# recursiveGecko/Formula-VAD

Measured on AMD Instinct MI355X. Metric: 20ms audio frames/sec end-to-end VAD pipeline, higher is better.
Workload: dtype f32

## Files before the change

### formula-vad_amd/csrc/engine.cpp

```cpp
#include <algorithm>
#include <cctype>
#include <cmath>
#include <cstdio>
#include <cstdlib>
#include <cstring>
#include <atomic>
#include <mutex>
#include <thread>

#include "internal.h"

#ifndef FVAD_DIAG
#define FVAD_DIAG 0
#endif

namespace fvad {

int set_err(const fvad_ctx* ctx, int code, const std::string& msg)
{
    if (ctx) ctx->err = msg;
    return code;
}
int hip_fail(const fvad_ctx* ctx, hipError_t e, const char* what)
{
// ... 60 lines not shown
                    if ((long long)p * p > m) p = m;
                }
                m /= p;
                if (nf >= 14) { hipFree(pd.d); return set_err(ctx, FVAD_ERR_INVALID_FFT_SIZE, "fft_size has too many prime factors"); }
                pd.plan.fac[nf++] = p;
            }
            pd.plan.n_fac = nf;
        }
        it = ctx->vad_plans.emplace(key, pd).first;
        ctx->ws.generation++;
    }
    *out = it->second.plan;
    return FVAD_OK;
}

static int apply_option(fvad_ctx* ctx, const std::string& name, const char* value)
{
    Tuning& tn = ctx->tune;
    const Tuning def;
    const bool unset = !value || !*value;
    const std::string v = unset ? "" : value;
    auto to_long = [&](long& out) { char* end = nullptr; out = strtol(v.c_str(), &end, 10); return end && *end == 0; };
    auto to_bool = [&](bool& out) { if (unset || v == "0") { out = false; return true; } if (v == "1") { out = true; return true; } return false; };
    if (name == "nn_math") {
        if (unset) tn.nn_math_force = -1;
        else if (v == "f32") tn.nn_math_force = FVAD_NN_MATH_F32;
        else if (v == "f16x3") tn.nn_math_force = FVAD_NN_MATH_F16X3;
        else if (v == "bf16x3") tn.nn_math_force = FVAD_NN_MATH_BF16X3;
        else return FVAD_ERR_INVALID_ARGUMENT;
    } else if (name == "gru_kernel") {
        if (!unset && v != "v3w12" && v != "v3w8" && v != "v3w4" && v != "v4w8" && v != "v5w0" && v != "v6w0") return FVAD_ERR_INVALID_ARGUMENT;
        tn.gru_kernel = v;
    } else if (name == "gemm_kernel") {
        if (!unset && v != "v1" && v != "v3" && v != "v3nofold") return FVAD_ERR_INVALID_ARGUMENT;
        tn.gemm_kernel = v;
    } else if (name == "h3_waves") {
        long w = 0;
        if (!unset && (!to_long(w) || (w != 0 && w != 8 && w != 12))) return FVAD_ERR_INVALID_ARGUMENT;
        tn.h3_waves = (int)w;
    } else if (name == "max_chunks") {
        long c = def.max_chunks;
        if (!unset && (!to_long(c) || c < 1)) return FVAD_ERR_INVALID_ARGUMENT;
        tn.max_chunks = c;
    } else if (name == "copy_threads") {
        long c = def.copy_threads;
        if (!unset && (!to_long(c) || c < 1 || c > 256)) return FVAD_ERR_INVALID_ARGUMENT;
        tn.copy_threads = (int)c;
    } else if (name == "ws_spin_ticks") {
        if (unset) { tn.ws_spin_ticks = def.ws_spin_ticks; tn.ws_spin_auto = true; }
        else {
            char* end = nullptr;
            tn.ws_spin_ticks = strtoull(v.c_str(), &end, 10);
            if (!end || *end) return FVAD_ERR_INVALID_ARGUMENT;
            tn.ws_spin_auto = false;
        }
    } else if (name == "ws2_variant") {
        long c = 0;
        if (!unset && (!to_long(c) || c < 0 || c >= (1 << 24))) return FVAD_ERR_INVALID_ARGUMENT;
#if !FVAD_DIAG
        if (c & (1 | 2 | 4 | 32 | 64 | 256 | 512 | 4096 | 8192 | 16384)) return FVAD_ERR_INVALID_ARGUMENT;
#endif
        tn.ws2_variant = (int)c;
    } else if (name == "ws2_waits") {
        long c = 0;
        if (!unset && (!to_long(c) || c < 0 || c > 0x7FFFFFFFL)) return FVAD_ERR_INVALID_ARGUMENT;
        tn.ws2_waits = (unsigned)c;
    } else if (name == "ws2_calibrate") {
// ... 655 lines not shown
```

### formula-vad_amd/csrc/kernels.h

```cpp
#pragma once
#include <hip/hip_runtime.h>
#include <stddef.h>
#include <stdint.h>

#include "../../include/fvad.h"

enum { FVAD_ACT_NONE = 0, FVAD_ACT_RELU = 1, FVAD_ACT_SIGMOID = 2 };

constexpr int kNFft = 320;
constexpr int kNHop = 160;
constexpr int kFramesPerChunk = 50;
constexpr int kWarmupRows = 4;
constexpr int kRowsPerChunk = kFramesPerChunk + kWarmupRows;
constexpr int kNBins = 161;
constexpr int kFeatStride = 176;
constexpr int kDown = 3;
constexpr int kChunk48 = kFramesPerChunk * kNHop * kDown;
constexpr int kVadFft = 1024;
constexpr int kVadFftMax = 16384;

struct LaneCarry {
    float in_tail[kNHop * kDown];
    float feat_tail[kWarmupRows * kNBins];
    float ola_tail[kNHop];
// ... 24 lines not shown
    const float* win320;
    const float* win320n;
    const float* tw160;
    const float* st320;
};

struct VadFftPlan {
    int n;
    const float* win;
    const float* tw;
    const float* st;
    float norm;
    int generic;
    int n_fac;
    int fac[14];
};

int fvad_launch_panel_gemm(const float* A, int lda, const float* Wfrag, const float* bias, float* C,
                           int ldc, long rows, int nt, int n_blocks, int S_steps, int act,
                           int map_T, int map_skip, hipStream_t stream, int n_valid_tiles = 0,
                           const unsigned* guard = nullptr);
struct GemmRowMap {
    int n_rows = 0, L = 0, in_T = 0, in_t0 = 0, out_T = 0, out_t0 = 0;
};
int fvad_launch_panel_gemm_s_rows(const float* A, int lda, const float* Wfrag, const float* bias, float* C, int ldc,
                                  GemmRowMap rm, int nt, int n_blocks, int S_steps, int act, hipStream_t stream,
                                  int n_valid_tiles = 0, const unsigned* guard = nullptr);
int fvad_launch_panel_gemm_s(const float* A, int lda, const float* Wfrag, const float* bias, float* C, int ldc,
                             long rows, int nt, int n_blocks, int S_steps, int act, int map_T, int map_skip,
                             hipStream_t stream, int n_valid_tiles = 0, const unsigned* guard = nullptr);
int fvad_launch_panel_gemm3(const float* A, int lda, const float* Wfrag, const float* bias, float* C,
                            int ldc, long rows, int nt, int n_blocks, int S_steps, int K, int act,
                            int n_valid_tiles, int map_T, int map_skip, int n_wg, hipStream_t stream);
int fvad_launch_panel_gemm_h3(const float* A, int in_ts, int a_ld, const float* Wfrag, const float* bias, float* C,
                              int out, int c_ld, int seq_T, long row_tiles, int nt, int n_blocks, int K, int act,
                              int n_valid_tiles, int map_T, int map_skip, float sx, float sw, float out_sx, int n_wg,
                              hipStream_t stream);
int fvad_launch_gru_rec_h3(const float* gi, const float* Rfrag, const float* bR, float* hsplit,
                           long n_seq_pad, int T, int waves, float sx, float sw, hipStream_t stream);
int fvad_launch_gru_ws2_fallback(float* gi, const float* feat, const float* W1frag_nt2, const float* bG1, const float* R1frag, const float* bR1,
                                 const float* W2frag_nt2, const float* bW2, const float* R2frag, const float* bR2, float* h1, float* h2,
                                 long n_seq_pad, int T, unsigned* sync, unsigned long long* fallbacks, hipStream_t stream,
                                 int zero_at = 0, int zero_n = 0);
int fvad_launch_gru_lat(const float* gi, const float* R2frag, const float* bR, float* hout,
                        long n_seq_pad, int T, const unsigned* guard, int tile_major, hipStream_t stream, int row_tiles = 1);
void fvad_launch_zero_words(unsigned* p, int n, hipStream_t stream);
void fvad_launch_count_word(unsigned long long* counter, const unsigned* word, hipStream_t stream);
bool fvad_gru_ws_shape(long n_seq_pad, int n_cu, int* RT, int* G);
size_t fvad_gru_ws_exchange_floats(long n_seq_pad);
int fvad_launch_gru_ws(const float* gi, const float* R2frag, const float* bR, float* hout, float* hx, unsigned* flags,
                       unsigned* err, long n_seq_pad, int T, int n_cu, int tile_major, unsigned long long spin_ticks,
                       hipStream_t stream);
bool fvad_gru_ws2_shape(long n_seq_pad, int n_cu, int* RT, int* G);
size_t fvad_gru_ws2_exchange_floats(long n_seq_pad);
bool fvad_gru_ws2_gi1_in_kernel(long n_seq_pad, int T, int n_cu, int variant);
bool fvad_gru_ws2_ok(long n_seq_pad, int T, int n_cu, int variant);
const char* fvad_gru_ws2_kernel_name(long n_seq_pad, int T, int n_cu, int variant);
int fvad_launch_gru_ws2(const float* gi1, const float* feat, const float* W1frag, const float* bG1, const float* R1frag, const float* bR1,
                        const float* W2frag, const float* bW2, const float* R2frag, const float* bR2, float* hout2, float* hx,
                        unsigned* flags, unsigned* err, long n_seq_pad, int T, int n_cu, unsigned long long spin_ticks, int variant,
                        unsigned waits, hipStream_t stream, unsigned* lsync = nullptr);
constexpr int kWs2LocalWords = 336;
bool fvad_gru_ws2_local_layer1(long n_seq_pad, int T, int n_cu, int variant);
int fvad_gru_ws2_wait_class(long n_seq_pad, int T, int n_cu, int variant);
unsigned fvad_gru_ws2_builtin_waits(int wait_class, bool local_layer1 = false);
int fvad_launch_gru_gen(const float* gi, int gi_ld, const float* R2frag, const float* bR, float* hout, int h_ld,
// ... 120 lines not shown
```

### formula-vad_amd/csrc/kernels_nn.hip

```cpp

#include <hip/hip_runtime.h>
#include <stdint.h>
#include <type_traits>

#include "kernels.h"

#include "nn_device.h"

__device__ __forceinline__ float act_sigmoid(float x) { return 1.0f / (1.0f + expf(-x)); }

template <int NT, int ACT, int WAVES>
__global__ __launch_bounds__(WAVES * 64) void panel_gemm_kernel(
    const float* __restrict__ A, int lda, const float* __restrict__ Wfrag,
    const float* __restrict__ bias, float* __restrict__ C, int ldc, int S_steps, int row_map_T,
    int row_map_skip, int n_valid_tiles, const unsigned* guard)
{
    __shared__ __attribute__((aligned(16))) float slab[2][NT * 256];
    if (guard && *guard == 0) return;

    const int tid = threadIdx.x;
    const int lane = tid & 63;
    const int wave = tid >> 6;
    const int m = lane & 15;
    const int q = lane >> 4;
// ... 250 lines not shown
                               bias, C, ldc, rm, n_valid_tiles, guard);                                              \
        else                                                                                                         \
            return -1;                                                                                               \
        return 0;                                                                                                    \
    }
    CASES(11, FVAD_ACT_NONE)
    CASES(25, FVAD_ACT_NONE)
    CASES(25, FVAD_ACT_RELU)
    CASES(38, FVAD_ACT_RELU)
    CASES(38, FVAD_ACT_SIGMOID)
#undef CASES
    return -1;
}

template <int T, int N> struct StaticFor {
    template <class F> static __device__ __forceinline__ void run(F&& f) {
        f(std::integral_constant<int, T>{});
        StaticFor<T + 1, N>::run(f);
    }
};
template <int N> struct StaticFor<N, N> {
    template <class F> static __device__ __forceinline__ void run(F&&) {}
};

template <int OFF> __device__ __forceinline__ void lds_read_b128(f32x4& dst, unsigned addr)
{
    asm volatile("ds_read_b128 %0, %1 offset:%2" : "=v"(dst) : "v"(addr), "n"(OFF));
}
template <int N> __device__ __forceinline__ void lds_wait(f32x4& dst)
{
    asm volatile("s_waitcnt lgkmcnt(%1)" : "+v"(dst) : "n"(N));
}

template <int NT, int RT, int ACT, int SP, int WAVES>
__global__ __launch_bounds__(WAVES * 64) __attribute__((amdgpu_waves_per_eu(2, 2))) void panel_gemm3_kernel(
    const float* __restrict__ A, int lda, const float* __restrict__ Wfrag,
    const float* __restrict__ bias, float* __restrict__ C, int ldc, int S_steps, int n_blocks,
    int n_valid_tiles, int row_map_T, int row_map_skip, unsigned n_items, int tail_r)
{
    __shared__ __attribute__((aligned(16))) float slab[2][NT * SP * 256];
    __shared__ __attribute__((aligned(16))) float sbias[2][NT * 16];
    typedef __attribute__((address_space(3))) float lds_float;

    const int tid = threadIdx.x;
    const int lane = tid & 63;
    const int wave = __builtin_amdgcn_readfirstlane(tid >> 6);
    const int m = lane & 15;
    const int q = lane >> 4;
    const int P = (S_steps + SP - 1) / SP;
    constexpr int WAITN = (NT - 1 < 15) ? NT - 1 : 15;

    auto a_pointer = [&](unsigned item, int rt) -> const float* {
        const unsigned panel = item / (unsigned)n_blocks;
        const unsigned row = ((panel * WAVES + wave) * RT + rt) * 16 + m;
        unsigned a_row = row;
        if (row_map_T > 0) {
            const unsigned per = (unsigned)(row_map_T - row_map_skip);
            const unsigned qd = row / per;
            a_row = qd * (unsigned)row_map_T + (unsigned)row_map_skip + (row - qd * per);
        }
        return A + (size_t)a_row * (size_t)lda + 4 * q;
    };
    auto issue = [&](unsigned item, int p, float* dst) {
        const int nblk = (int)(item % (unsigned)n_blocks);
        const int s0 = p * SP;
        const int cnt = (S_steps - s0 < SP) ? (S_steps - s0) : SP;
        const float* src = Wfrag + ((size_t)nblk * S_steps + s0) * (NT * 256);
// ... 13 lines not shown
    };

    unsigned item = (gridDim.x % 8u == 0u) ? (blockIdx.x % 8u) * (gridDim.x / 8u) + blockIdx.x / 8u : blockIdx.x;
    if (item >= n_items) return;
    const unsigned slab_addr[2] = {(unsigned)(uintptr_t)(lds_float*)slab[0] + (unsigned)lane * 16u,
                                   (unsigned)(uintptr_t)(lds_float*)slab[1] + (unsigned)lane * 16u};
    typedef const __attribute__((address_space(1))) f32x4* gptr4;
    const float* a_ptr[RT];
    f32x4 a0[RT], apre[RT];
#pragma unroll
    for (int rt = 0; rt < RT; ++rt) {
        a_ptr[rt] = a_pointer(item, rt);
        a0[rt] = *(gptr4)(a_ptr[rt]);
        apre[rt] = *(gptr4)(a_ptr[rt] + 16);
    }
    issue(item, 0, slab[0]);
    stage_bias(item, sbias[0]);
    __syncthreads();
    int buf = 0, bbuf = 0;

    for (; item < n_items; item += gridDim.x) {
        const unsigned next_item = item + gridDim.x;
        const bool has_next = next_item < n_items;
        f32x4 acc[RT][NT];
        {
            const f32x4* bl = reinterpret_cast<const f32x4*>(sbias[bbuf]) + q;
#pragma unroll
            for (int t = 0; t < NT; ++t) {
                const f32x4 b4 = bl[4 * t];
#pragma unroll
                for (int rt = 0; rt < RT; ++rt) acc[rt][t] = b4;
            }
        }
        const float* a_nextitem[RT];
#pragma unroll
        for (int rt = 0; rt < RT; ++rt) a_nextitem[rt] = has_next ? a_pointer(next_item, rt) : a_ptr[rt];

        for (int p = 0; p < P; ++p) {
            const int s0 = p * SP;
            const int cnt = (S_steps - s0 < SP) ? (S_steps - s0) : SP;
            if (p + 1 < P) issue(item, p + 1, slab[buf ^ 1]);
            else if (has_next) { issue(next_item, 0, slab[buf ^ 1]); stage_bias(next_item, sbias[bbuf ^ 1]); }

            unsigned rd = slab_addr[buf];
            f32x4 w[NT];
            StaticFor<0, NT>::run([&](auto tc) {
                constexpr int t = decltype(tc)::value;
                lds_read_b128<t * 1024>(w[t], rd);
            });
            auto super_step = [&](int s, auto last_c) {
                constexpr bool LAST = decltype(last_c)::value;
                const int sg = s0 + s;
                f32x4 a1[RT];
                if (sg == 0) {
#pragma unroll
                    for (int rt = 0; rt < RT; ++rt) a1[rt] = apre[rt];
                } else {
#pragma unroll
                    for (int rt = 0; rt < RT; ++rt)
                        a1[rt] = *(gptr4)((sg + 1 < S_steps) ? a_ptr[rt] + 16 * (sg + 1) : a_nextitem[rt]);
                }
                const int nr = (sg + 1 < S_steps) ? 4 : tail_r;
                auto mfmas = [&](auto tc) {
                    constexpr int t = decltype(tc)::value;
#pragma unroll
                    for (int rt = 0; rt < RT; ++rt) acc[rt][t] = MFMA16(w[t].x, a0[rt].x, acc[rt][t]);
                    if (nr > 1) {
#pragma unroll
                        for (int rt = 0; rt < RT; ++rt) acc[rt][t] = MFMA16(w[t].y, a0[rt].y, acc[rt][t]);
                    }
                    if (nr > 2) {
#pragma unroll
                        for (int rt = 0; rt < RT; ++rt) acc[rt][t] = MFMA16(w[t].z, a0[rt].z, acc[rt][t]);
                    }
                    if (nr > 3) {
#pragma unroll
                        for (int rt = 0; rt < RT; ++rt) acc[rt][t] = MFMA16(w[t].w, a0[rt].w, acc[rt][t]);
                    }
                };
                StaticFor<0, NT>::run([&](auto tc) {
                    constexpr int t = decltype(tc)::value;
                    if constexpr (LAST) {
                        lds_wait<((NT - 1 - t) < 15 ? (NT - 1 - t) : 15)>(w[t]);
                        mfmas(tc);
                    } else {
                        lds_wait<WAITN>(w[t]);
                        mfmas(tc);
                        lds_read_b128<(NT + t) * 1024>(w[t], rd);
                    }
                });
                rd += NT * 1024;
#pragma unroll
                for (int rt = 0; rt < RT; ++rt) a0[rt] = a1[rt];
            };
            for (int s = 0; s + 1 < cnt; ++s) super_step(s, std::false_type{});
            super_step(cnt - 1, std::true_type{});
            __syncthreads();
// ... 25 lines not shown
            o.z = __int_as_float(__builtin_amdgcn_ds_bpermute(bp_addr, __float_as_int(v[2])));
            o.w = __int_as_float(__builtin_amdgcn_ds_bpermute(bp_addr, __float_as_int(v[3])));
            *reinterpret_cast<f32x4*>(c_ptr[rt] + 16 * t) = o;
        };
        if (valid_t >= NT) {
#pragma unroll
            for (int t = 0; t < NT; ++t)
#pragma unroll
                for (int rt = 0; rt < RT; ++rt) emit(t, rt);
        } else {
#pragma unroll
            for (int t = 0; t < NT; ++t) {
                if (t < valid_t) {
#pragma unroll
                    for (int rt = 0; rt < RT; ++rt) emit(t, rt);
                }
            }
        }
        bbuf ^= 1;
#pragma unroll
        for (int rt = 0; rt < RT; ++rt) a_ptr[rt] = a_nextitem[rt];
    }
}

int fvad_launch_panel_gemm3(const float* A, int lda, const float* Wfrag, const float* bias, float* C,
                            int ldc, long rows, int nt, int n_blocks, int S_steps, int K, int act,
                            int n_valid_tiles, int map_T, int map_skip, int n_wg, hipStream_t stream)
{
    if (rows % 256) return -1;
    const int n_last = K - 16 * (S_steps - 1);
    const int tail_r = n_last >= 4 ? 4 : (n_last < 1 ? 4 : n_last);
    const unsigned n_items = (unsigned)((rows / 256) * n_blocks);
    const unsigned grid = n_items < (unsigned)n_wg ? n_items : (unsigned)n_wg;
#define CASE3(NT_, ACT_, SP_)                                                                         \
    if (nt == NT_ && act == ACT_) {                                                                   \
        hipLaunchKernelGGL((panel_gemm3_kernel<NT_, 2, ACT_, SP_, 8>), dim3(grid), dim3(512), 0, stream, \
                           A, lda, Wfrag, bias, C, ldc, S_steps, n_blocks, n_valid_tiles, map_T,      \
                           map_skip, n_items, tail_r);                                                \
        return 0;                                                                                     \
    }
    CASE3(15, FVAD_ACT_NONE, 5)
    CASE3(13, FVAD_ACT_RELU, 5)
    CASE3(11, FVAD_ACT_SIGMOID, 6)
#undef CASE3
    return -1;
}


template <int WAVES>
__device__ __forceinline__ void gru3_issue_slab(const float* __restrict__ src, float* lds_dst, int wave, unsigned lane16)
{
    asm volatile("" : "+v"(lane16));
#pragma unroll
    for (int b = wave; b < 3 * GRU_J; b += WAVES) {
        __builtin_amdgcn_global_load_lds(
            (const __attribute__((address_space(1))) void*)((const __attribute__((address_space(1))) char*)src + b * 1024 + lane16),
            (__attribute__((address_space(3))) void*)(lds_dst + b * 256), 16, 0, 0);
    }
}

template <int WAVES, int D, bool TS3>
__global__ __launch_bounds__(WAVES * 64) void gru_rec3_kernel(const float* __restrict__ gi,
                                                              const float* __restrict__ R2frag,
                                                              const float* __restrict__ bR,
                                                              float* hout, int T, float* hs3)
{
    __shared__ __attribute__((aligned(16))) float slab[2][GRU2_SLAB];
    typedef __attribute__((address_space(3))) float lds_float;

    const int tid = threadIdx.x;
    const int lane = tid & 63;
    const int wave = __builtin_amdgcn_readfirstlane(tid >> 6);
    const int m = lane & 15;
    const int q = lane >> 4;
    typedef const __attribute__((address_space(1))) char* gbytes;
    const size_t seq0 = (size_t)(blockIdx.x * WAVES + wave) * 16;
    gbytes gi_w = (gbytes)(gi + seq0 * T * (3 * GRU_H));
// ... 548 lines not shown
```

### formula-vad_amd/csrc/nn_dispatch.cpp

```cpp
#include <algorithm>
#include <atomic>
#include <cmath>
#include <cstdio>
#include <cstdlib>
#include <cstring>
#include <mutex>
#include <thread>

#include "internal.h"

namespace fvad {

void free_workspace_nn(Workspace& ws)
{
    float** bufs[] = {&ws.feat, &ws.spec, &ws.a1, &ws.gi, &ws.h1, &ws.h2, &ws.hs1, &ws.hs2, &ws.f2, &ws.f3, &ws.gains};
    for (float** b : bufs) { if (*b) hipFree(*b); *b = nullptr; }
    if (ws.descs) hipFree(ws.descs);
    if (ws.h_descs) hipHostFree(ws.h_descs);
    ws.descs = nullptr; ws.h_descs = nullptr;
    ws.descs_mirror.clear();
    ws.cap_chunks = 0;
    ws.cap_rows = 0;
    ws.a1_cap_rows = ws.h_cap_rows = ws.hs_cap_rows = 0;
}
// ... 292 lines not shown
    auto S = [](int K) { return (K + 15) / 16; };
    int rc = 0;
    ctx->last_nn_path = "f32: panel_gemm<8> + gru_gen (model dims " + std::to_string(g.F1) + "/" + std::to_string(g.H) + "/" +
                        std::to_string(g.N2) + "/" + std::to_string(g.N3) + ")";
    time_begin(ctx, "fc1_gemm");
    rc |= fvad_launch_panel_gemm(ws.feat, kFeatStride, m.g_fc1_w.p, m.g_fc1_b.p, ws.a1, g.F1p, rows, 8, g.F1p / 128, S(161), FVAD_ACT_NONE, 0, 0, st);
    time_end(ctx);
    time_begin(ctx, "gru1_in_gemm");
    rc |= fvad_launch_panel_gemm(ws.a1, g.F1p, m.g_gi1_w.p, m.g_gi1_b.p, ws.gi, g.Gp, rows, 8, g.Gp / 128, S(g.F1), FVAD_ACT_NONE, 0, 0, st);
    time_end(ctx);
    time_begin(ctx, "gru1_rec");
    rc |= fvad_launch_gru_gen(ws.gi, g.Gp, m.g_r1.p, m.g_br1.p, ws.h1, g.Hp, n_pad, T, g.J, st);
    time_end(ctx);
    time_begin(ctx, "gru2_in_gemm");
    rc |= fvad_launch_panel_gemm(ws.h1, g.Hp, m.g_gi2_w.p, m.g_gi2_b.p, ws.gi, g.Gp, rows, 8, g.Gp / 128, g.J, FVAD_ACT_NONE, 0, 0, st);
    time_end(ctx);
    time_begin(ctx, "gru2_rec");
    rc |= fvad_launch_gru_gen(ws.gi, g.Gp, m.g_r2.p, m.g_br2.p, ws.h2, g.Hp, n_pad, T, g.J, st);
    time_end(ctx);
    time_begin(ctx, "fc2_gemm");
    rc |= fvad_launch_panel_gemm(ws.h2, g.Hp, m.g_fc2_w.p, m.g_fc2_b.p, ws.f2, g.N2p, rows_out, 8, g.N2p / 128, g.J, FVAD_ACT_RELU, skip ? T : 0, skip, st);
    time_end(ctx);
    time_begin(ctx, "fc3_gemm");
    rc |= fvad_launch_panel_gemm(ws.f2, g.N2p, m.g_fc3_w.p, m.g_fc3_b.p, ws.f3, g.N3p, rows_out, 8, g.N3p / 128, S(g.N2), FVAD_ACT_RELU, 0, 0, st);
    time_end(ctx);
    time_begin(ctx, "fc4_gemm");
    rc |= fvad_launch_panel_gemm(ws.f3, g.N3p, m.g_fc4_w.p, m.g_fc4_b.p, ws.gains, kFeatStride, rows_out, 11, 1, S(g.N3), FVAD_ACT_SIGMOID, 0, 0, st);
    time_end(ctx);
    if (rc) return set_err(ctx, FVAD_ERR_INVALID_ARGUMENT, "no kernel instance for this layer shape");
    FVAD_HIP(ctx, hipGetLastError());
    return FVAD_OK;
}

int run_nn(fvad_ctx* ctx, long n_pad, int T, int skip, long n_real)
{
    if (!ctx->dm.loaded) return set_err(ctx, FVAD_ERR_NO_MODEL, "NSNet2 weights not loaded");
    if (n_real <= 0 || n_real > n_pad) n_real = n_pad;
    if (ctx->dm.generic) return run_nn_generic(ctx, n_pad, T, skip);
    Workspace& ws = ctx->ws;
    const DeviceModel& m = ctx->dm;
    hipStream_t st = ctx->stream;
    const long rows = n_pad * T;
    const long rows_out = n_pad * (T - skip);
    int rc = 0;
    const Tuning& tn = ctx->tune;
    const char* force = tn.gemm_kernel.empty() ? nullptr : tn.gemm_kernel.c_str();
    const int math = nn_math_effective(ctx);
    const bool h3 = math == FVAD_NN_MATH_F16X3, b3 = math == FVAD_NN_MATH_BF16X3;
    if ((h3 || b3) && n_pad % 128) return set_err(ctx, FVAD_ERR_INVALID_ARGUMENT, "the emulated kernels need a batch padded to 128 sequences");
    {
        const size_t r = (size_t)rows;
        const bool nofold = force && strstr(force, "nofold");
        if (r > ws.cap_rows || (h3 ? r > ws.hs_cap_rows : r > ws.h_cap_rows) || (nofold && r > ws.a1_cap_rows))
            return set_err(ctx, FVAD_ERR_INVALID_ARGUMENT, "NSNet2 workspace not allocated for this arithmetic / batch");
    }
    if (b3) {
        if (!ws.b3_hs1 || (size_t)n_pad * (size_t)T > ws.b3_cap_rows) return set_err(ctx, FVAD_ERR_INVALID_ARGUMENT, "bf16x3 workspace not allocated");
        auto gemm_b3 = [&](const float* A, int in_ts, int a_ld, const DevBuf& W, const float* b, float* Cc, int out, int c_ld, int seq_T,
                           long row_tiles, int nt, int nblk, int K, int act, int valid, int mT, int mskip) {
            return fvad_launch_panel_gemm_b3(A, in_ts, a_ld, W.p, b, Cc, out, c_ld, seq_T, row_tiles, nt, nblk, K, act, valid, mT, mskip, ctx->n_cu, st);
        };
        const int waves = n_pad % 192 == 0 ? 12 : 8;
        const long G = n_pad / 16;
        ctx->last_nn_path = std::string("bf16x3: panel_gemm_b3 (fc1 folded) + gru_rec3<") + std::to_string(waves) + "> (f32 recurrences)";
        time_begin(ctx, "gru1_in_gemm_fc1folded");
        rc |= gemm_b3(ws.feat, 0, kFeatStride, m.gi1f_b3, m.gi1f_bzr.p, ws.gi, 0, 1200, T, G * T, 15, 5, 161, FVAD_ACT_NONE, 75, 0, 0);
        time_end(ctx);
        time_begin(ctx, "gru1_rec");
        rc |= fvad_launch_gru_rec3(ws.gi, m.r1v2.p, m.br1.p, ws.h1, n_pad, T, waves, st, ws.b3_hs1);
        time_end(ctx);
        time_begin(ctx, "gru2_in_gemm");
        rc |= gemm_b3(ws.b3_hs1, 1, 13, m.gi2_b3, m.gi2_bzr.p, ws.gi, 0, 1200, T, G * T, 15, 5, 400, FVAD_ACT_NONE, 75, 0, 0);
        time_end(ctx);
        time_begin(ctx, "gru2_rec");
        rc |= fvad_launch_gru_rec3(ws.gi, m.r2v2.p, m.br2.p, ws.h2, n_pad, T, waves, st, ws.b3_hs2);
        time_end(ctx);
        time_begin(ctx, "fc2_gemm");
        rc |= gemm_b3(ws.b3_hs2, 1, 13, m.fc2_b3, m.fc2h3_b.p, ws.b3_f2, 2, 19, T - skip, G * (T - skip), 10, 4, 400, FVAD_ACT_RELU, 38, skip ? T : 0, skip);
        time_end(ctx);
        time_begin(ctx, "fc3_gemm");
        rc |= gemm_b3(ws.b3_f2, 1, 19, m.fc3_b3, m.fc3h3_b.p, ws.b3_f3, 2, 19, T - skip, G * (T - skip), 10, 4, 600, FVAD_ACT_RELU, 38, 0, 0);
        time_end(ctx);
        time_begin(ctx, "fc4_gemm");
        rc |= gemm_b3(ws.b3_f3, 1, 19, m.fc4_b3, m.fc4h3_b.p, ws.gains, 0, kFeatStride, T - skip, G * (T - skip), 12, 1, 600, FVAD_ACT_SIGMOID, 11, 0, 0);
        time_end(ctx);
        if (rc) return set_err(ctx, FVAD_ERR_INVALID_ARGUMENT, "no kernel instance for this layer shape");
        FVAD_HIP(ctx, hipGetLastError());
        return FVAD_OK;
    }
    const bool big = h3 || (force ? force[1] != '1' : (tn.reproducible || n_pad >= 2048));
    if (tn.reproducible && !force && (rows % 256 || rows_out % 256))
        return set_err(ctx, FVAD_ERR_INVALID_ARGUMENT, "reproducible: batch not padded to the persistent GEMM's 256-row panels");
    if (big && rows % 256 == 0 && rows_out % 256 == 0) {
        auto gemm = [&](const float* A, int lda, const float* W, const float* b, float* Cc, int ldc, long r, int nt,
                        int nblk, int S, int K, int act, int valid, int mT, int mskip) {
            return fvad_launch_panel_gemm3(A, lda, W, b, Cc, ldc, r, nt, nblk, S, K, act, valid, mT, mskip, ctx->n_cu, st);
        };
        auto gemm_h3 = [&](const float* A, int in_ts, int a_ld, const DevBuf& W, const DeviceModel::H3Scale& sc, const float* b,
                           float* Cc, int out, int c_ld, int seq_T, long row_tiles, int nt, int nblk, int K, int act,
                           int valid, int mT, int mskip, float out_sx) {
            return fvad_launch_panel_gemm_h3(A, in_ts, a_ld, W.p, b, Cc, out, c_ld, seq_T, row_tiles, nt, nblk, K, act, valid,
                                             mT, mskip, sc.sx, sc.sw, out_sx, ctx->n_cu, st);
        };
        if (h3) {
            int waves = n_pad % 192 == 0 ? 12 : 8;
            if ((tn.h3_waves == 8 || tn.h3_waves == 12) && n_pad % (16 * tn.h3_waves) == 0) waves = tn.h3_waves;
            ctx->last_nn_path = std::string("f16x3: panel_gemm_h3 + gru_rec_h3<") + std::to_string(waves) + ">";
            const long G = n_pad / 16;
            time_begin(ctx, "gru1_in_gemm_fc1folded");
            rc |= gemm_h3(ws.feat, 0, kFeatStride, m.gi1f_h3, m.h3_gi1f, m.gi1f_bzr.p, ws.gi, 1, 75, T, G * T, 15, 5, 161, FVAD_ACT_NONE, 75, 0, 0, 1.0f);
            time_end(ctx);
            time_begin(ctx, "gru1_rec");
            rc |= fvad_launch_gru_rec_h3(ws.gi, m.r1_h3.p, m.br1.p, ws.hs1, n_pad, T, waves, m.h3_r1.sx, m.h3_r1.sw, st);
            time_end(ctx);
            time_begin(ctx, "gru2_in_gemm");
            rc |= gemm_h3(ws.hs1, 1, 13, m.gi2_h3, m.h3_gi2, m.gi2_bzr.p, ws.gi, 1, 75, T, G * T, 15, 5, 400, FVAD_ACT_NONE, 75, 0, 0, 1.0f);
            time_end(ctx);
            time_begin(ctx, "gru2_rec");
            rc |= fvad_launch_gru_rec_h3(ws.gi, m.r2_h3.p, m.br2.p, ws.hs2, n_pad, T, waves, m.h3_r2.sx, m.h3_r2.sw, st);
            time_end(ctx);
            time_begin(ctx, "fc2_gemm");
            rc |= gemm_h3(ws.hs2, 1, 13, m.fc2_h3, m.h3_fc2, m.fc2h3_b.p, ws.f2, 2, 19, T - skip, G * (T - skip), 10, 4, 400, FVAD_ACT_RELU, 38, skip ? T : 0, skip, m.h3_fc3.sx);
            time_end(ctx);
            time_begin(ctx, "fc3_gemm");
            rc |= gemm_h3(ws.f2, 1, 19, m.fc3_h3, m.h3_fc3, m.fc3h3_b.p, ws.f3, 2, 19, T - skip, G * (T - skip), 10, 4, 600, FVAD_ACT_RELU, 38, 0, 0, m.h3_fc4.sx);
            time_end(ctx);
            time_begin(ctx, "fc4_gemm");
            rc |= gemm_h3(ws.f3, 1, 19, m.fc4_h3, m.h3_fc4, m.fc4h3_b.p, ws.gains, 0, kFeatStride, T - skip, G * (T - skip), 12, 1, 600, FVAD_ACT_SIGMOID, 11, 0, 0, 1.0f);
            time_end(ctx);
            if (rc) return set_err(ctx, FVAD_ERR_INVALID_ARGUMENT, "no kernel instance for this layer shape");
            FVAD_HIP(ctx, hipGetLastError());
            return FVAD_OK;
        }
        const bool fold = !(force && strstr(force, "nofold"));
        const GruChoice gc = pick_gru(ctx, n_pad, T, fold);
        ctx->last_nn_path = std::string("f32: panel_gemm3") + (fold ? " (fc1 folded)" : "") + " + " +
                            (gc.version == 3 ? "gru_rec3<" + std::to_string(gc.waves) + ">" : gc.version == 5 ? std::string("gru_ws") : std::string("gru_lat"));
        if (gc.version == 5 && (rc = prepare_gru_ws(ctx, n_pad))) return rc;
        const bool bzr = gc.version == 3;
        if (fold) {
            time_begin(ctx, "gru1_in_gemm_fc1folded");
            rc |= gemm(ws.feat, kFeatStride, m.gi1f_w.p, bzr ? m.gi1f_bzr.p : m.gi1f_b.p, ws.gi, 1200, rows, 15, 5, 11, 161, FVAD_ACT_NONE, 75, 0, 0);
            time_end(ctx);
        } else {
            time_begin(ctx, "fc1_gemm");
            rc |= fvad_launch_panel_gemm(ws.feat, kFeatStride, m.fc1_w.p, m.fc1_b.p, ws.a1, 400, rows, 25, 1, 11, FVAD_ACT_NONE, 0, 0, st);
            time_end(ctx);
            time_begin(ctx, "gru1_in_gemm");
            rc |= gemm(ws.a1, 400, m.gi1v2_w.p, m.gi1_btm.p, ws.gi, 1200, rows, 15, 5, 25, 400, FVAD_ACT_NONE, 75, 0, 0);
            time_end(ctx);
        }
        time_begin(ctx, "gru1_rec");
        rc |= launch_gru(ctx, gc, ws.gi, m.r1v2, m.br1.p, ws.h1, n_pad, T, 0, 1);
        time_end(ctx);
        time_begin(ctx, "gru2_in_gemm");
        rc |= gemm(ws.h1, 400, m.gi2v2_w.p, bzr ? m.gi2_bzr.p : m.gi2_btm.p, ws.gi, 1200, rows, 15, 5, 25, 400, FVAD_ACT_NONE, 75, 0, 0);
        time_end(ctx);
        time_begin(ctx, "gru2_rec");
        rc |= launch_gru(ctx, gc, ws.gi, m.r2v2, m.br2.p, ws.h2, n_pad, T, 1, 1);
        time_end(ctx);
        time_begin(ctx, "fc2_gemm");
        rc |= gemm(ws.h2, 400, m.fc2v3_w.p, m.fc2v3_b.p, ws.f2, 608, rows_out, 13, 3, 25, 400, FVAD_ACT_RELU, 38, skip ? T : 0, skip);
        time_end(ctx);
        time_begin(ctx, "fc3_gemm");
        rc |= gemm(ws.f2, 608, m.fc3v3_w.p, m.fc3v3_b.p, ws.f3, 608, rows_out, 13, 3, 38, 600, FVAD_ACT_RELU, 38, 0, 0);
        time_end(ctx);
        time_begin(ctx, "fc4_gemm");
        rc |= gemm(ws.f3, 608, m.fc4_w.p, m.fc4_b.p, ws.gains, kFeatStride, rows_out, 11, 1, 38, 600, FVAD_ACT_SIGMOID, 11, 0, 0);
        time_end(ctx);
        if (rc) return set_err(ctx, FVAD_ERR_INVALID_ARGUMENT, "no kernel instance for this layer shape");
        FVAD_HIP(ctx, hipGetLastError());
        return FVAD_OK;
    }
    const int fam = rows > 2048 ? 1 : 0, snt = fam ? 4 : 2;
    const int nb_gi = (75 + snt - 1) / snt, nb_fc = (38 + snt - 1) / snt;
    const GruChoice gcs = pick_gru(ctx, n_pad, T, false);
    const bool gi1_in_kernel = gcs.version == 6 && fvad_gru_ws2_gi1_in_kernel(n_pad, T, ctx->n_cu, tn.ws2_variant);
    if (!gi1_in_kernel) {
        time_begin(ctx, "gru1_in_gemm_fc1folded");
        rc |= fvad_launch_panel_gemm_s(ws.feat, kFeatStride, m.s_gi1f_w[fam].p, m.gi1f_b.p, ws.gi, 1200, rows, snt, nb_gi, 11, FVAD_ACT_NONE, 0, 0, st, 75);
        time_end(ctx);
    }
    if (gcs.version >= 5 && (rc = prepare_gru_ws(ctx, n_pad))) return rc;
    ctx->last_nn_path = std::string("f32: panel_gemm (fc1 folded) + ") + (gcs.version == 6 ? fvad_gru_ws2_kernel_name(n_pad, T, ctx->n_cu, tn.ws2_variant) :
                        gcs.version == 5 ? "gru_ws" : "gru_lat");
    if (gcs.version == 6) {
        unsigned* err = ws.ws_sync + 512;
        time_begin(ctx, "gru12_rec_pipelined");
        rc |= ws_serialised(ctx, [&] {
            return fvad_launch_gru_ws2(ws.gi, ws.feat, m.s_w1frag.p, m.gi1f_b.p, m.r1v2.p, m.br1.p, m.s_w2frag.p, m.s_bw2.p, m.r2v2.p, m.br2.p, ws.h2,
                                       ws.hx, ws.ws_sync, err, n_pad, T, ctx->n_cu, ws_spin_deadline(ctx, gru_ws2_cost_both_layers(n_pad, T, ctx->n_cu, tn.ws2_variant) * T / 55.0), tn.ws2_variant,
                                       tn.ws2_waits ? tn.ws2_waits : tn.ws2_waits_cal[fvad_gru_ws2_wait_class(n_pad, T, ctx->n_cu, tn.ws2_variant)], st,
                                       ws.ws_sync + kWsLocalAt);
        });
        rc |= fvad_launch_gru_ws2_fallback(ws.gi, gi1_in_kernel ? ws.feat : nullptr, m.s_gi1f_w[0].p, m.gi1f_b.p, m.r1v2.p, m.br1.p, m.s_gi2_w[0].p,
                                           m.gi2_btm.p, m.r2v2.p, m.br2.p, ws.h1, ws.h2, n_pad, T, ws.ws_sync, ws.ws_fallbacks, st, (int)kWsLocalAt, kWs2LocalWords);
        {
            hipStreamCaptureStatus cap = hipStreamCaptureStatusNone;
            (void)hipStreamIsCapturing(st, &cap);
            if (rc == 0 && cap == hipStreamCaptureStatusNone) ws.sync_clean = true;
        }
        time_end(ctx);
// ... 228 lines not shown
            ws.descs_mirror.assign(hd, hd + n);
        }
        time_begin(ctx, "stft320_logpow");
        const int fft_parts = n <= 85 ? 3 : (n <= 128 ? 2 : 1);
        fvad_launch_stft(dd, (int)n, ctx->tb, ws.feat, ws.spec, ctx->stream, fft_parts);
        time_end(ctx);
        for (const Tap& t : taps) {
            const LaneJob& lj = jobs[t.job];
            if (lj.h_spec)
                FVAD_HIP(ctx, hipMemcpyAsync(lj.h_spec + t.chunk0 * (size_t)(kFramesPerChunk * kNBins * 2),
                                             ws.spec + (size_t)t.batch0 * (kFramesPerChunk * kNBins * 2),
                                             t.count * (size_t)(kFramesPerChunk * kNBins * 2) * sizeof(float), hipMemcpyDeviceToHost, ctx->stream));
            if (lj.h_feat)
                FVAD_HIP(ctx, hipMemcpy2DAsync(lj.h_feat + t.chunk0 * (size_t)(kRowsPerChunk * kNBins), kNBins * sizeof(float),
                                               ws.feat + (size_t)t.batch0 * (kRowsPerChunk * kFeatStride), kFeatStride * sizeof(float),
                                               kNBins * sizeof(float), t.count * (size_t)kRowsPerChunk, hipMemcpyDeviceToHost, ctx->stream));
        }
        const long n_pad = padded_batch(ctx, n, kRowsPerChunk, kWarmupRows);
        rc = run_nn(ctx, n_pad, kRowsPerChunk, kWarmupRows, n);
        if (rc) return rc;
        time_begin(ctx, "istft320_ola_up3");
        fvad_launch_istft(dd, (int)n, ctx->tb, ws.spec, ws.gains, kFramesPerChunk, 0, ctx->stream, fft_parts);
        time_end(ctx);
        for (size_t t : touched) jobs[t].cur ^= 1;
        if (n_launches) ++*n_launches;
        job = j;
        chunk_in_job = c;
    }
    FVAD_HIP(ctx, hipGetLastError());
    return FVAD_OK;
}

}
```

Before: 25.05 million.

## Add weight-resident persistent GEMM with balanced panel split for fc1-folded GRU input

Adds a persistent GEMM kernel that loads one column block of weight fragments into LDS once per workgroup and then streams row panels through it. A host-side split spreads workgroups over column blocks in proportion to their tile counts and gives each workgroup a strided set of panels. By default this is used only for the fc1-folded GRU1 input GEMM. It is meant to remove repeated weight reloads from global memory and to balance work across CUs, at the cost of more LDS use and more complex launch logic. The fc2/fc3 panel_gemm3 instance also skips MFMAs on the padding tile in the last block.

```diff
diff --git a/formula-vad_amd/csrc/engine.cpp b/formula-vad_amd/csrc/engine.cpp
--- a/formula-vad_amd/csrc/engine.cpp
+++ b/formula-vad_amd/csrc/engine.cpp
@@ -116,7 +116,7 @@
         if (!unset && v != "v3w12" && v != "v3w8" && v != "v3w4" && v != "v4w8" && v != "v5w0" && v != "v6w0") return FVAD_ERR_INVALID_ARGUMENT;
         tn.gru_kernel = v;
     } else if (name == "gemm_kernel") {
-        if (!unset && v != "v1" && v != "v3" && v != "v3nofold") return FVAD_ERR_INVALID_ARGUMENT;
+        if (!unset && v != "v1" && v != "v3" && v != "v3nofold" && v != "v4" && v != "v4nofold") return FVAD_ERR_INVALID_ARGUMENT;
         tn.gemm_kernel = v;
     } else if (name == "h3_waves") {
         long w = 0;
diff --git a/formula-vad_amd/csrc/kernels.h b/formula-vad_amd/csrc/kernels.h
--- a/formula-vad_amd/csrc/kernels.h
+++ b/formula-vad_amd/csrc/kernels.h
@@ -80,6 +80,17 @@
 int fvad_launch_panel_gemm3(const float* A, int lda, const float* Wfrag, const float* bias, float* C,
                             int ldc, long rows, int nt, int n_blocks, int S_steps, int K, int act,
                             int n_valid_tiles, int map_T, int map_skip, int n_wg, hipStream_t stream);
+constexpr int FVAD_RES_MAX_WG = 320;
+struct GemmResSplit {
+    unsigned p0[FVAD_RES_MAX_WG];
+    unsigned short cnt[FVAD_RES_MAX_WG];
+    unsigned char blk[FVAD_RES_MAX_WG], stride[FVAD_RES_MAX_WG];
+};
+bool fvad_gemm_res_split(GemmResSplit& sp, long n_panels, const int* w, int n_blocks, int n_wg);
+int fvad_panel_gemm_res_rows(int K, int n_valid_tiles, int act);
+int fvad_launch_panel_gemm_res(const float* A, int lda, const float* Wfrag, int src_nt, const float* bias, float* C, int ldc,
+                               long rows, int K, int act, int n_valid_tiles, int map_T, int map_skip, int n_wg,
+                               hipStream_t stream);
 int fvad_launch_panel_gemm_h3(const float* A, int in_ts, int a_ld, const float* Wfrag, const float* bias, float* C,
                               int out, int c_ld, int seq_T, long row_tiles, int nt, int n_blocks, int K, int act,
                               int n_valid_tiles, int map_T, int map_skip, float sx, float sw, float out_sx, int n_wg,
diff --git a/formula-vad_amd/csrc/kernels_nn.hip b/formula-vad_amd/csrc/kernels_nn.hip
--- a/formula-vad_amd/csrc/kernels_nn.hip
+++ b/formula-vad_amd/csrc/kernels_nn.hip
@@ -306,7 +306,7 @@
     asm volatile("s_waitcnt lgkmcnt(%1)" : "+v"(dst) : "n"(N));
 }
 
-template <int NT, int RT, int ACT, int SP, int WAVES>
+template <int NT, int RT, int ACT, int SP, int WAVES, int NTS = NT>
 __global__ __launch_bounds__(WAVES * 64) __attribute__((amdgpu_waves_per_eu(2, 2))) void panel_gemm3_kernel(
     const float* __restrict__ A, int lda, const float* __restrict__ Wfrag,
     const float* __restrict__ bias, float* __restrict__ C, int ldc, int S_steps, int n_blocks,
@@ -386,6 +386,7 @@
                 for (int rt = 0; rt < RT; ++rt) acc[rt][t] = b4;
             }
         }
+        const bool skip_pad = NTS != NT && n_valid_tiles - (int)(item % (unsigned)n_blocks) * NT == NTS;
         const float* a_nextitem[RT];
 #pragma unroll
         for (int rt = 0; rt < RT; ++rt) a_nextitem[rt] = has_next ? a_pointer(next_item, rt) : a_ptr[rt];
@@ -417,6 +418,7 @@
                 const int nr = (sg + 1 < S_steps) ? 4 : tail_r;
                 auto mfmas = [&](auto tc) {
                     constexpr int t = decltype(tc)::value;
+                    if (t >= NTS && skip_pad) return;
 #pragma unroll
                     for (int rt = 0; rt < RT; ++rt) acc[rt][t] = MFMA16(w[t].x, a0[rt].x, acc[rt][t]);
                     if (nr > 1) {
@@ -508,17 +510,290 @@
     const int tail_r = n_last >= 4 ? 4 : (n_last < 1 ? 4 : n_last);
     const unsigned n_items = (unsigned)((rows / 256) * n_blocks);
     const unsigned grid = n_items < (unsigned)n_wg ? n_items : (unsigned)n_wg;
-#define CASE3(NT_, ACT_, SP_)                                                                         \
+#define CASE3(NT_, ACT_, SP_, NTS_)                                                                       \
     if (nt == NT_ && act == ACT_) {                                                                   \
-        hipLaunchKernelGGL((panel_gemm3_kernel<NT_, 2, ACT_, SP_, 8>), dim3(grid), dim3(512), 0, stream, \
+        hipLaunchKernelGGL((panel_gemm3_kernel<NT_, 2, ACT_, SP_, 8, NTS_>), dim3(grid), dim3(512), 0, stream, \
                            A, lda, Wfrag, bias, C, ldc, S_steps, n_blocks, n_valid_tiles, map_T,      \
                            map_skip, n_items, tail_r);                                                \
         return 0;                                                                                     \
     }
-    CASE3(15, FVAD_ACT_NONE, 5)
-    CASE3(13, FVAD_ACT_RELU, 5)
-    CASE3(11, FVAD_ACT_SIGMOID, 6)
+    CASE3(15, FVAD_ACT_NONE, 5, 15)
+    CASE3(13, FVAD_ACT_RELU, 5, 12)
+    CASE3(11, FVAD_ACT_SIGMOID, 6, 11)
 #undef CASE3
+    return -1;
+}
+
+template <int OFF> __device__ __forceinline__ void lds_read_b32(float& dst, unsigned addr)
+{
+    asm volatile("ds_read_b32 %0, %1 offset:%2" : "=v"(dst) : "v"(addr), "n"(OFF));
+}
+template <int N> __device__ __forceinline__ void lds_wait(float& dst)
+{
+    asm volatile("s_waitcnt lgkmcnt(%1)" : "+v"(dst) : "n"(N));
+}
+
+template <int NT, int NTL, int RT, int ACT, int S, int TAIL_R>
+__global__ __launch_bounds__(512) __attribute__((amdgpu_waves_per_eu(2, 2))) void panel_gemm_res_kernel(
+    const float* __restrict__ A, int lda, const float* __restrict__ Wfrag, int src_nt,
+    const float* __restrict__ bias, float* __restrict__ C, int ldc, int n_blocks, int row_map_T, int row_map_skip,
+    GemmResSplit sp)
+{
+    constexpr int WAVES = 8;
+    constexpr bool TAILQ = TAIL_R == 1;
+    constexpr int FULL = TAILQ ? S - 1 : S;
+    static_assert(NT <= 15 && NTL >= 1 && NTL <= NT && FULL >= 2, "lgkmcnt is a 4-bit field; the ring needs two full steps");
+    static_assert((2 * NT - 1) * 1024 < 65536, "ds_read offset field");
+    __shared__ __attribute__((aligned(16))) float wres[FULL * NT * 256 + (TAILQ ? NT * 64 : 0)];
+    __shared__ __attribute__((aligned(16))) float sbias[NT * 16];
+    typedef __attribute__((address_space(3))) float lds_float;
+    typedef const __attribute__((address_space(1))) f32x4* gptr4;
+
+    const int tid = threadIdx.x;
+    const int lane = tid & 63;
+    const int wave = __builtin_amdgcn_readfirstlane(tid >> 6);
+    const int m = lane & 15;
+    const int q = lane >> 4;
+
+    asm volatile("" ::: "a0");
+    const unsigned slot = (gridDim.x % 8u == 0u) ? (blockIdx.x % 8u) * (gridDim.x / 8u) + blockIdx.x / 8u : blockIdx.x;
+    const unsigned cnt = sp.cnt[slot];
+    if (cnt == 0) return;
+    const int nblk = sp.blk[slot];
+    const unsigned stride = sp.stride[slot];
+    const unsigned p_first = sp.p0[slot];
+    const int ntv = (nblk == n_blocks - 1) ? NTL : NT;
+
+    for (int idx = tid; idx < FULL * NT * 64; idx += WAVES * 64) {
+        const int fb = idx >> 6, s = fb / NT, t = fb - s * NT;
+        const int tile = nblk * NT + t, sb = tile / src_nt, st = tile - sb * src_nt;
+        if (t < ntv)
+            reinterpret_cast<f32x4*>(wres)[idx] =
+                reinterpret_cast<const f32x4*>(Wfrag)[((size_t)(sb * S + s) * src_nt + st) * 64 + (idx & 63)];
+    }
+    if (TAILQ) {
+        for (int idx = tid; idx < NT * 64; idx += WAVES * 64) {
+            const int t = idx >> 6;
+            const int tile = nblk * NT + t, sb = tile / src_nt, st = tile - sb * src_nt;
+            if (t < ntv) wres[FULL * NT * 256 + idx] = Wfrag[(((size_t)(sb * S + S - 1) * src_nt + st) * 64 + (idx & 63)) * 4];
+        }
+    }
+    if (tid < ntv * 4) reinterpret_cast<f32x4*>(sbias)[tid] = reinterpret_cast<const f32x4*>(bias + nblk * (NT * 16))[tid];
+    __syncthreads();
+
+    auto a_pointer = [&](unsigned panel, int rt) -> const float* {
+        const unsigned row = ((panel * WAVES + wave) * RT + rt) * 16 + m;
+        unsigned a_row = row;
+        if (row_map_T > 0) {
+            const unsigned per = (unsigned)(row_map_T - row_map_skip);
+            const unsigned qd = row / per;
+            a_row = qd * (unsigned)row_map_T + (unsigned)row_map_skip + (row - qd * per);
+        }
+        return A + (size_t)a_row * (size_t)lda + 4 * q;
+    };
+
+    auto body = [&](auto ntv_c) {
+        constexpr int NTV = decltype(ntv_c)::value;
+        const unsigned base = (unsigned)(uintptr_t)(lds_float*)wres + (unsigned)lane * 16u;
+        const unsigned tbase = (unsigned)(uintptr_t)(lds_float*)(wres + FULL * NT * 256) + (unsigned)lane * 4u;
+        unsigned panel = p_first;
+        const float* a_ptr[RT];
+        f32x4 a0[RT], apre[RT];
+#pragma unroll
+        for (int rt = 0; rt < RT; ++rt) {
+            a_ptr[rt] = a_pointer(panel, rt);
+            a0[rt] = *(gptr4)(a_ptr[rt]);
+            apre[rt] = *(gptr4)(a_ptr[rt] + 16);
+        }
+        f32x4 w[NTV];
+        float wt[NTV];
+        StaticFor<0, NTV>::run([&](auto tc) {
+            constexpr int t = decltype(tc)::value;
+            lds_read_b128<t * 1024>(w[t], base);
+        });
+
+        for (unsigned i = 0; i < cnt; ++i, panel += stride) {
+            const bool has_next = i + 1 < cnt;
+            f32x4 acc[RT][NTV];
+            {
+                unsigned boff = (unsigned)q;
+                asm volatile("" : "+v"(boff));
+                const f32x4* bl = reinterpret_cast<const f32x4*>(sbias) + boff;
+#pragma unroll
+                for (int t = 0; t < NTV; ++t) {
+                    const f32x4 b4 = bl[4 * t];
+#pragma unroll
+                    for (int rt = 0; rt < RT; ++rt) acc[rt][t] = b4;
+                }
+            }
+            unsigned rd = base;
+            auto super_step = [&](int sg, auto mode_c) {
+                constexpr int MODE = decltype(mode_c)::value;
+                constexpr int NR = MODE == 2 ? TAIL_R : 4;
+                f32x4 a1[RT];
+                if (sg == 0) {
+#pragma unroll
+                    for (int rt = 0; rt < RT; ++rt) a1[rt] = apre[rt];
+                } else {
+#pragma unroll
+                    for (int rt = 0; rt < RT; ++rt) a1[rt] = *(gptr4)(MODE == 2 ? a_ptr[rt] : a_ptr[rt] + 16 * (sg + 1));
+                }
+                StaticFor<0, NTV>::run([&](auto tc) {
+                    constexpr int t = decltype(tc)::value;
+                    if constexpr (MODE == 2 && TAILQ) lds_wait<NTV - 1>(wt[t]);
+                    else lds_wait<NTV - 1>(w[t]);
+                    const float wx = (MODE == 2 && TAILQ) ? wt[t] : w[t].x;
+#pragma unroll
+                    for (int rt = 0; rt < RT; ++rt) acc[rt][t] = MFMA16(wx, a0[rt].x, acc[rt][t]);
+                    if constexpr (NR > 1) {
+#pragma unroll
+                        for (int rt = 0; rt < RT; ++rt) acc[rt][t] = MFMA16(w[t].y, a0[rt].y, acc[rt][t]);
+                    }
+                    if constexpr (NR > 2) {
+#pragma unroll
+                        for (int rt = 0; rt < RT; ++rt) acc[rt][t] = MFMA16(w[t].z, a0[rt].z, acc[rt][t]);
+                    }
+                    if constexpr (NR > 3) {
+#pragma unroll
+                        for (int rt = 0; rt < RT; ++rt) acc[rt][t] = MFMA16(w[t].w, a0[rt].w, acc[rt][t]);
+                    }
+                    if constexpr (MODE == 0) lds_read_b128<(NT + t) * 1024>(w[t], rd);
+                    else if constexpr (MODE == 1) lds_read_b32<t * 256>(wt[t], tbase);
+                    else lds_read_b128<t * 1024>(w[t], base);
+                });
+                if (MODE == 0) rd += NT * 1024;
+#pragma unroll
+                for (int rt = 0; rt < RT; ++rt) a0[rt] = a1[rt];
+            };
+            constexpr int N0 = TAILQ ? S - 2 : S - 1;
+            for (int s = 0; s < N0; ++s) super_step(s, std::integral_constant<int, 0>{});
+            if (TAILQ) super_step(S - 2, std::integral_constant<int, 1>{});
+            if (has_next) {
+#pragma unroll
+                for (int rt = 0; rt < RT; ++rt) a_ptr[rt] = a_pointer(panel + stride, rt);
+            }
+            super_step(S - 1, std::integral_constant<int, 2>{});
+
+#pragma unroll
+            for (int rt = 0; rt < RT; ++rt) apre[rt] = *(gptr4)(a_ptr[rt] + 16);
+            const int bp_addr = ((lane >> 2) + 16 * (lane & 3)) * 4;
+            float* c_ptr[RT];
+#pragma unroll
+            for (int rt = 0; rt < RT; ++rt) {
+                const unsigned row = ((panel * WAVES + wave) * RT + rt) * 16 + (unsigned)(lane >> 2);
+                c_ptr[rt] = C + (size_t)row * (size_t)ldc + nblk * (NT * 16) + 4 * (lane & 3);
+            }
+#pragma unroll
+            for (int t = 0; t < NTV; ++t) {
+#pragma unroll
+                for (int rt = 0; rt < RT; ++rt) {
+                    f32x4 v = acc[rt][t];
+                    if (ACT == FVAD_ACT_RELU) {
+                        v.x = fmaxf(v.x, 0.f); v.y = fmaxf(v.y, 0.f); v.z = fmaxf(v.z, 0.f); v.w = fmaxf(v.w, 0.f);
+                    } else if (ACT == FVAD_ACT_SIGMOID) {
+                        v.x = act_sigmoid(v.x); v.y = act_sigmoid(v.y); v.z = act_sigmoid(v.z); v.w = act_sigmoid(v.w);
+                    }
+                    f32x4 o;
+                    o.x = __int_as_float(__builtin_amdgcn_ds_bpermute(bp_addr, __float_as_int(v[0])));
+                    o.y = __int_as_float(__builtin_amdgcn_ds_bpermute(bp_addr, __float_as_int(v[1])));
+                    o.z = __int_as_float(__builtin_amdgcn_ds_bpermute(bp_addr, __float_as_int(v[2])));
+                    o.w = __int_as_float(__builtin_amdgcn_ds_bpermute(bp_addr, __float_as_int(v[3])));
+                    *reinterpret_cast<f32x4*>(c_ptr[rt] + 16 * t) = o;
+                }
+            }
+        }
+        StaticFor<0, NTV>::run([&](auto tc) { lds_wait<0>(w[decltype(tc)::value]); });
+    };
+    if (NTL != NT && ntv != NT) body(std::integral_constant<int, NTL>{});
+    else body(std::integral_constant<int, NT>{});
+}
+
+bool fvad_gemm_res_split(GemmResSplit& sp, long n_panels, const int* w, int n_blocks, int n_wg)
+{
+    if (n_wg > FVAD_RES_MAX_WG || n_blocks < 1 || n_blocks > n_wg || n_blocks > 255 || n_panels <= 0) return false;
+    int N[256], k_next[256];
+    for (int b = 0; b < n_blocks; ++b) { N[b] = 1; k_next[b] = 0; }
+    for (int i = n_blocks; i < n_wg; ++i) {
+        int best = 0;
+        for (int b = 1; b < n_blocks; ++b)
+            if ((long)w[b] * N[best] > (long)w[best] * N[b]) best = b;
+        ++N[best];
+    }
+    int blk_of[FVAD_RES_MAX_WG], k_of[FVAD_RES_MAX_WG];
+    for (int i = 0; i < n_wg; ++i) {
+        int best = -1;
+        for (int b = 0; b < n_blocks; ++b) {
+            if (k_next[b] >= N[b]) continue;
+            if (best < 0 || (long)(2 * k_next[b] + 1) * N[best] < (long)(2 * k_next[best] + 1) * N[b]) best = b;
+        }
+        blk_of[i] = best;
+        k_of[i] = k_next[best]++;
+    }
+    const int nx = n_wg % 8 == 0 ? 8 : 1, per_x = n_wg / nx;
+    for (int x = 0; x < nx; ++x) {
+        int k0[256], n[256];
+        for (int b = 0; b < n_blocks; ++b) { k0[b] = -1; n[b] = 0; }
+        for (int i = x * per_x; i < (x + 1) * per_x; ++i) {
+            if (k0[blk_of[i]] < 0) k0[blk_of[i]] = k_of[i];
+            ++n[blk_of[i]];
+        }
+        for (int i = x * per_x; i < (x + 1) * per_x; ++i) {
+            const int b = blk_of[i], j = k_of[i] - k0[b];
+            const long lo = n_panels * k0[b] / N[b], hi = n_panels * (k0[b] + n[b]) / N[b];
+            const long len = hi - lo, c = len > j ? (len - j + n[b] - 1) / n[b] : 0;
+            if (c > 65535 || n[b] > 255) return false;
+            sp.p0[i] = (unsigned)(lo + j);
+            sp.cnt[i] = (unsigned short)c;
+            sp.blk[i] = (unsigned char)b;
+            sp.stride[i] = (unsigned char)n[b];
+        }
+    }
+    return true;
+}
+
+namespace {
+struct ResInstance { int K, tiles, act, nt, ntl, rt; };
+constexpr ResInstance kResInstances[] = {
+    {161, 75, FVAD_ACT_NONE, 15, 15, 2},
+    {400, 75, FVAD_ACT_NONE, 5, 5, 6},
+    {400, 38, FVAD_ACT_RELU, 5, 3, 6},
+};
+const ResInstance* res_instance(int K, int n_valid_tiles, int act)
+{
+    for (const ResInstance& r : kResInstances)
+        if (r.K == K && r.tiles == n_valid_tiles && r.act == act) return &r;
+    return nullptr;
+}
+}
+
+int fvad_panel_gemm_res_rows(int K, int n_valid_tiles, int act)
+{
+    const ResInstance* r = res_instance(K, n_valid_tiles, act);
+    return r ? 8 * r->rt * 16 : 0;
+}
+
+int fvad_launch_panel_gemm_res(const float* A, int lda, const float* Wfrag, int src_nt, const float* bias, float* C, int ldc,
+                               long rows, int K, int act, int n_valid_tiles, int map_T, int map_skip, int n_wg,
+                               hipStream_t stream)
+{
+    const ResInstance* r = res_instance(K, n_valid_tiles, act);
+    if (!r || rows <= 0 || rows % (8 * r->rt * 16)) return -1;
+    const int n_blocks = (n_valid_tiles + r->nt - 1) / r->nt;
+    int w[16];
+    for (int b = 0; b < n_blocks; ++b) w[b] = b + 1 < n_blocks ? r->nt : r->ntl;
+    if (n_wg > FVAD_RES_MAX_WG) n_wg = FVAD_RES_MAX_WG - FVAD_RES_MAX_WG % 8;
+    GemmResSplit sp;
+    if (n_wg < n_blocks || !fvad_gemm_res_split(sp, rows / (8 * r->rt * 16), w, n_blocks, n_wg)) return -1;
+#define CASE_RES(NT_, NTL_, RT_, ACT_, S_, TAIL_)                                                                    \
+    if (r->nt == NT_ && r->ntl == NTL_ && act == ACT_) {                                                             \
+        hipLaunchKernelGGL((panel_gemm_res_kernel<NT_, NTL_, RT_, ACT_, S_, TAIL_>), dim3(n_wg), dim3(512), 0, stream, A, lda, \
+                           Wfrag, src_nt, bias, C, ldc, n_blocks, map_T, map_skip, sp);                              \
+        return 0;                                                                                                    \
+    }
+    CASE_RES(15, 15, 2, FVAD_ACT_NONE, 11, 1)
+    CASE_RES(5, 5, 6, FVAD_ACT_NONE, 25, 4)
+    CASE_RES(5, 3, 6, FVAD_ACT_RELU, 25, 4)
+#undef CASE_RES
     return -1;
 }
 
diff --git a/formula-vad_amd/csrc/nn_dispatch.cpp b/formula-vad_amd/csrc/nn_dispatch.cpp
--- a/formula-vad_amd/csrc/nn_dispatch.cpp
+++ b/formula-vad_amd/csrc/nn_dispatch.cpp
@@ -348,6 +348,8 @@
     return FVAD_OK;
 }
 
+static bool res_by_default(const char* layer) { return strcmp(layer, "gi1f") == 0; }
+
 int run_nn(fvad_ctx* ctx, long n_pad, int T, int skip, long n_real)
 {
     if (!ctx->dm.loaded) return set_err(ctx, FVAD_ERR_NO_MODEL, "NSNet2 weights not loaded");
@@ -408,8 +410,15 @@
     if (tn.reproducible && !force && (rows % 256 || rows_out % 256))
         return set_err(ctx, FVAD_ERR_INVALID_ARGUMENT, "reproducible: batch not padded to the persistent GEMM's 256-row panels");
     if (big && rows % 256 == 0 && rows_out % 256 == 0) {
-        auto gemm = [&](const float* A, int lda, const float* W, const float* b, float* Cc, int ldc, long r, int nt,
+        const bool v4 = force && force[1] == '4';
+        std::string res_layers;
+        auto gemm = [&](const char* layer, const float* A, int lda, const float* W, const float* b, float* Cc, int ldc, long r, int nt,
                         int nblk, int S, int K, int act, int valid, int mT, int mskip) {
+            const bool want = force ? v4 : res_by_default(layer);
+            if (want && fvad_launch_panel_gemm_res(A, lda, W, nt, b, Cc, ldc, r, K, act, valid, mT, mskip, ctx->n_cu, st) == 0) {
+                res_layers += std::string(res_layers.empty() ? "" : ", ") + layer;
+                return 0;
+            }
             return fvad_launch_panel_gemm3(A, lda, W, b, Cc, ldc, r, nt, nblk, S, K, act, valid, mT, mskip, ctx->n_cu, st);
         };
         auto gemm_h3 = [&](const float* A, int in_ts, int a_ld, const DevBuf& W, const DeviceModel::H3Scale& sc, const float* b,
@@ -450,40 +459,41 @@
         }
         const bool fold = !(force && strstr(force, "nofold"));
         const GruChoice gc = pick_gru(ctx, n_pad, T, fold);
-        ctx->last_nn_path = std::string("f32: panel_gemm3") + (fold ? " (fc1 folded)" : "") + " + " +
-                            (gc.version == 3 ? "gru_rec3<" + std::to_string(gc.waves) + ">" : gc.version == 5 ? std::string("gru_ws") : std::string("gru_lat"));
+        const std::string gru_name = gc.version == 3 ? "gru_rec3<" + std::to_string(gc.waves) + ">" : gc.version == 5 ? std::string("gru_ws") : std::string("gru_lat");
         if (gc.version == 5 && (rc = prepare_gru_ws(ctx, n_pad))) return rc;
         const bool bzr = gc.version == 3;
         if (fold) {
             time_begin(ctx, "gru1_in_gemm_fc1folded");
-            rc |= gemm(ws.feat, kFeatStride, m.gi1f_w.p, bzr ? m.gi1f_bzr.p : m.gi1f_b.p, ws.gi, 1200, rows, 15, 5, 11, 161, FVAD_ACT_NONE, 75, 0, 0);
+            rc |= gemm("gi1f", ws.feat, kFeatStride, m.gi1f_w.p, bzr ? m.gi1f_bzr.p : m.gi1f_b.p, ws.gi, 1200, rows, 15, 5, 11, 161, FVAD_ACT_NONE, 75, 0, 0);
             time_end(ctx);
         } else {
             time_begin(ctx, "fc1_gemm");
             rc |= fvad_launch_panel_gemm(ws.feat, kFeatStride, m.fc1_w.p, m.fc1_b.p, ws.a1, 400, rows, 25, 1, 11, FVAD_ACT_NONE, 0, 0, st);
             time_end(ctx);
             time_begin(ctx, "gru1_in_gemm");
-            rc |= gemm(ws.a1, 400, m.gi1v2_w.p, m.gi1_btm.p, ws.gi, 1200, rows, 15, 5, 25, 400, FVAD_ACT_NONE, 75, 0, 0);
+            rc |= gemm("gi1", ws.a1, 400, m.gi1v2_w.p, m.gi1_btm.p, ws.gi, 1200, rows, 15, 5, 25, 400, FVAD_ACT_NONE, 75, 0, 0);
             time_end(ctx);
         }
         time_begin(ctx, "gru1_rec");
         rc |= launch_gru(ctx, gc, ws.gi, m.r1v2, m.br1.p, ws.h1, n_pad, T, 0, 1);
         time_end(ctx);
         time_begin(ctx, "gru2_in_gemm");
-        rc |= gemm(ws.h1, 400, m.gi2v2_w.p, bzr ? m.gi2_bzr.p : m.gi2_btm.p, ws.gi, 1200, rows, 15, 5, 25, 400, FVAD_ACT_NONE, 75, 0, 0);
+        rc |= gemm("gi2", ws.h1, 400, m.gi2v2_w.p, bzr ? m.gi2_bzr.p : m.gi2_btm.p, ws.gi, 1200, rows, 15, 5, 25, 400, FVAD_ACT_NONE, 75, 0, 0);
         time_end(ctx);
         time_begin(ctx, "gru2_rec");
         rc |= launch_gru(ctx, gc, ws.gi, m.r2v2, m.br2.p, ws.h2, n_pad, T, 1, 1);
         time_end(ctx);
         time_begin(ctx, "fc2_gemm");
-        rc |= gemm(ws.h2, 400, m.fc2v3_w.p, m.fc2v3_b.p, ws.f2, 608, rows_out, 13, 3, 25, 400, FVAD_ACT_RELU, 38, skip ? T : 0, skip);
+        rc |= gemm("fc2", ws.h2, 400, m.fc2v3_w.p, m.fc2v3_b.p, ws.f2, 608, rows_out, 13, 3, 25, 400, FVAD_ACT_RELU, 38, skip ? T : 0, skip);
         time_end(ctx);
         time_begin(ctx, "fc3_gemm");
-        rc |= gemm(ws.f2, 608, m.fc3v3_w.p, m.fc3v3_b.p, ws.f3, 608, rows_out, 13, 3, 38, 600, FVAD_ACT_RELU, 38, 0, 0);
+        rc |= gemm("fc3", ws.f2, 608, m.fc3v3_w.p, m.fc3v3_b.p, ws.f3, 608, rows_out, 13, 3, 38, 600, FVAD_ACT_RELU, 38, 0, 0);
         time_end(ctx);
         time_begin(ctx, "fc4_gemm");
-        rc |= gemm(ws.f3, 608, m.fc4_w.p, m.fc4_b.p, ws.gains, kFeatStride, rows_out, 11, 1, 38, 600, FVAD_ACT_SIGMOID, 11, 0, 0);
-        time_end(ctx);
+        rc |= gemm("fc4", ws.f3, 608, m.fc4_w.p, m.fc4_b.p, ws.gains, kFeatStride, rows_out, 11, 1, 38, 600, FVAD_ACT_SIGMOID, 11, 0, 0);
+        time_end(ctx);
+        ctx->last_nn_path = std::string("f32: panel_gemm3") + (res_layers.empty() ? "" : " / panel_gemm_res [" + res_layers + "]") +
+                            (fold ? " (fc1 folded)" : "") + " + " + gru_name;
         if (rc) return set_err(ctx, FVAD_ERR_INVALID_ARGUMENT, "no kernel instance for this layer shape");
         FVAD_HIP(ctx, hipGetLastError());
         return FVAD_OK;
@@ -778,3 +788,23 @@
 }
 
 }
+
+extern "C" int fvad_debug_nn_buffer(fvad_ctx* ctx, const char* name, void** ptr, size_t* cap_rows, int* ld)
+{
+    if (!ctx || !name || !ptr || !cap_rows || !ld) return FVAD_ERR_INVALID_ARGUMENT;
+    const fvad::Workspace& ws = ctx->ws;
+    if (!strcmp(name, "f2")) { *ptr = ws.f2; *ld = 608; }
+    else if (!strcmp(name, "f3")) { *ptr = ws.f3; *ld = 608; }
+    else return FVAD_ERR_INVALID_ARGUMENT;
+    *cap_rows = ws.cap_rows;
+    return FVAD_OK;
+}
+extern "C" long fvad_debug_padded_batch(const fvad_ctx* ctx, long n, int T, int skip) { return ctx ? fvad::padded_batch(ctx, n, T, skip) : -1; }
+extern "C" int fvad_debug_gemm_res_split(long n_panels, const int* w, int n_blocks, int n_wg, unsigned* p0, unsigned* cnt,
+                                         unsigned* blk, unsigned* stride)
+{
+    GemmResSplit sp;
+    if (!fvad_gemm_res_split(sp, n_panels, w, n_blocks, n_wg)) return -1;
+    for (int i = 0; i < n_wg; ++i) { p0[i] = sp.p0[i]; cnt[i] = sp.cnt[i]; blk[i] = sp.blk[i]; stride[i] = sp.stride[i]; }
+    return 0;
+}
```

Result: no change. 25.23 million, median of 6 (+0.7%).
